# laboshinl/loam_velodyne

Measured on AMD Instinct MI355X. Metric: sweeps/sec (64-ring, 1M-pt map): feature extraction + odometry + scan-to-map registration, higher is better.
Workload: dtype f32

## Files before the change

### loam_velodyne_amd/csrc/gn_iter_kernel.inc

```
__global__ __launch_bounds__(LX_RES_THREADS) __attribute__((amdgpu_waves_per_eu(GN_WAVES, GN_WAVES))) void GN_KERNEL(const GnArgs A) {
  constexpr int TRS = GN_TILE + 1;
  __shared__ uint32_t s_raw[(36 * GN_TILE > LX_NSUM * TRS) ? 36 * GN_TILE : LX_NSUM * TRS];
  float* tr = (float*)s_raw;
  uint32_t* s_tab = s_raw;
  __shared__ uint32_t s_nb[5 * GN_TILE];
  __shared__ double red[8][LX_NSUM];
  __shared__ int sh_last;
  const uint32_t s = blockIdx.y;
  if (A.stats[s].done) return;
  if (A.skip_word && *A.skip_word == A.skip_value) return;
  const int tid = (int)threadIdx.x;
  const uint32_t q0 = A.ds_off[2 * s], qm = A.ds_off[2 * s + 1], q1 = A.ds_off[2 * s + 2];
  const uint32_t tc = (qm - q0 + GN_TILE - 1) / GN_TILE, tsf = (q1 - qm + GN_TILE - 1) / GN_TILE;
  const uint32_t ntiles = (tc + tsf) ? tc + tsf : 1u;
  uint32_t tile;
  {
    const uint32_t x = blockIdx.x % 8, j = blockIdx.x / 8;
    const uint32_t tsurf = ntiles - tc;
    const uint32_t c0 = x * tc / 8, c1 = (x + 1) * tc / 8, s0 = x * tsurf / 8, s1 = (x + 1) * tsurf / 8;
    if (j < c1 - c0) tile = c0 + j;
    else if (j - (c1 - c0) < s1 - s0) tile = tc + s0 + (j - (c1 - c0));
    else return;
  }
  const bool corner = tile < tc;
  const uint32_t qbase = corner ? q0 + tile * GN_TILE : qm + (tile - tc) * GN_TILE;
  const uint32_t qend = corner ? qm : q1;
  GN_TS(0);
  const Pose T = A.poses[s];
  {
    const int grp = tid / KNN_LPQ, gl = tid % KNN_LPQ;
    const uint32_t q = qbase + (uint32_t)grp;
    if (q < qend) {
      const float4 po = A.ds_pts[q];
      float qx = po.x, qy = po.y, qz = po.z;
      to_map(T, qx, qy, qz);
      unsigned long long wk[6];
      uint32_t win[6];
      knn5_group<KNN_LPQ, GN_TILE>(corner ? *A.cdesc : *A.sdesc, corner ? A.cpts : A.spts, corner ? A.cstart : A.sstart, qx, qy, qz, gl, s_tab + grp, wk,
                                   win);
      if (gl == 0) {
        const float d5 = wk[4] != KNN_NONE ? __uint_as_float((uint32_t)(wk[4] >> 32)) : FLT_MAX;
#pragma unroll
        for (int j = 0; j < 5; j++) s_nb[j * GN_TILE + grp] = (j == 4 && !(d5 < 1.0f)) ? 0xffffffffu : win[j];
      }
    }
  }
// ... 70 lines not shown
```

### loam_velodyne_amd/csrc/odometry.hip

```cpp
#include "odometry.hpp"
#include "odom_schedule.hpp"
#include "pinned_copy.hpp"
#include <chrono>
#include <cstring>
#include <type_traits>

namespace loamx {

constexpr int OD_THREADS = 256;
constexpr int OD_TR_STRIDE = OD_THREADS + 2;
constexpr int OD_PART_STRIDE = 2 * (2 * 16 * LX_NSUM) + 16;
[[maybe_unused]] constexpr int OD_PART_TS = 2 * (2 * 16 * LX_NSUM);

__device__ inline void sincos_f(float a, float& s, float& c) { sincosf(a, &s, &c); }

__device__ inline void transform_to_start(const float* T, float scan_period, const float4 pi, float& x, float& y, float& z) {
  const float s = (1.f / scan_period) * (pi.w - (float)(int)pi.w);
  x = pi.x - s * T[3];
  y = pi.y - s * T[4];
  z = pi.z - s * T[5];
  float sx, cx, sy, cy, sz, cz;
  sincos_f(-s * T[0], sx, cx);
  sincos_f(-s * T[1], sy, cy);
  sincos_f(-s * T[2], sz, cz);
// ... 162 lines not shown
    const uint32_t w = __float_as_uint(p.w);
    if (valid && (d2 < lbest || (d2 == lbest && lw != 0xffffffffu && (w & OD_IDX_MASK) < (lw & OD_IDX_MASK)))) { lbest = d2; lw = w; }
  });
  float d = lbest;
  int j = lw == 0xffffffffu ? -1 : (int)(lw & OD_IDX_MASK), o_ = lw == 0xffffffffu ? 0x7fffffff : (int)(lw & OD_IDX_MASK);
  int ring = (int)(lw >> 24);
  {
#pragma unroll
    for (int off = 32; off > 0; off >>= 1) {
      const float od = __shfl_xor(d, off, 64);
      const int oj = __shfl_xor(j, off, 64), oo = __shfl_xor(o_, off, 64), orr = __shfl_xor(ring, off, 64);
      if (od < d || (od == d && oo < o_)) { d = od; j = oj; o_ = oo; ring = orr; }
    }
  }
  const float h = 1.0f / g.inv_h;
  if (j >= 0 && d < 25.0f && d <= h * h) { w_out = ((uint32_t)ring << 24) | (uint32_t)j; return j; }
  const int id = nn1_shells(g, sorted, cell_start, qx, qy, qz, lane, 2, (j >= 0 && d < 25.0f) ? d : 25.0f, (j >= 0 && d < 25.0f) ? j : -1);
  w_out = id == j ? (((uint32_t)ring << 24) | (uint32_t)j) : (0xff000000u | (uint32_t)(id < 0 ? 0 : id));
  return id;
}

#ifdef LOAMX_PROF_CORR
__device__ unsigned long long g_corr_ts[3][16];
#define OC_TS(k) do { if (blockIdx.y == 0 && lane == 0 && ts_slot >= 0) g_corr_ts[ts_slot][k] = wall_clock64(); } while (0)
#else
#define OC_TS(k) do { } while (0)
#endif
__global__ __launch_bounds__(256) OD_CORR_ATTR void k_odom_corr_grid(OdomProblem* __restrict__ probs, OdomParams P, uint32_t* __restrict__ patch_dst, uint4 patch) {
  if (patch_dst && blockIdx.x == 0 && blockIdx.y == 0 && threadIdx.x == 0) { patch_dst[0] = patch.x; patch_dst[1] = patch.y; patch_dst[2] = patch.z; }
  OdomProblem& pb = probs[blockIdx.y];
  if (pb.done) return;
  const int lane = threadIdx.x & 63, wid = threadIdx.x >> 6;
  const int nSharp = (int)pb.n_sharp, nFlat = (int)pb.n_flat;
  int f;
  {
    const int x = (int)(blockIdx.x % 8), j = (int)(blockIdx.x / 8);
    const int sS = (int)((long long)x * nSharp / 8), nS = (int)((long long)(x + 1) * nSharp / 8) - sS;
    const int sF = (int)((long long)x * nFlat / 8), nF = (int)((long long)(x + 1) * nFlat / 8) - sF;
    const int fl = 4 * j + wid;
    if (fl >= nS + nF) return;
    f = fl < nS ? sS + fl : nSharp + sF + (fl - nS);
  }
#ifdef LOAMX_PROF_CORR
  const int ts_slot = f == nSharp / 2 ? 0 : f == nSharp + nFlat / 2 ? 1 : f == nSharp + nFlat - 1 ? 2 : -1;
#endif
  OC_TS(0);
  float T[6];
#pragma unroll
  for (int k = 0; k < 6; k++) T[k] = pb.transform[k];
  const bool corner = f < nSharp;
  const float4 pi = corner ? pb.sharp[f] : pb.flat[f - nSharp];
  const uint32_t* __restrict__ tbl = corner ? pb.rf_corner : pb.rf_surf;
  const int e0 = max((int)pi.w - 8, 0);
  uint32_t tv = 0u, unordered_epoch = 0u;
  if (tbl) {
    if (e0 + lane < OD_RF_N - 1) tv = tbl[e0 + lane];
    unordered_epoch = tbl[OD_RF_N - 1];
  }
  float x, y, z;
  transform_to_start(T, P.scan_period, pi, x, y, z);
  const GridDescB gd = corner ? *pb.lc_desc : *pb.ls_desc;
  const float4* __restrict__ sorted = pb.sorted;
  const uint32_t* __restrict__ cell_start = pb.cell_table + gd.cell_base;
  OC_TS(1);
  Block27 B;
  block27_build(gd.g, cell_start, x, y, z, lane, B);
  OC_TS(2);
  uint32_t wbest = 0u;
  Block27First first;
  const int closest = nn1_block(gd.g, B, sorted, cell_start, x, y, z, lane, wbest, first);
  OC_TS(3);
  if (closest < 0) {
    if (lane == 0) { pb.ind[5 * f] = -1; pb.ind[5 * f + 1] = -1; pb.ind[5 * f + 2] = -1; }
    return;
  }
  const float4* last = corner ? pb.last_corner : pb.last_surf;
  const int nLast = corner ? (int)pb.n_last_corner : (int)pb.n_last_surf;
  const int nCur = corner ? nSharp : nFlat;
  const int bound = nCur < nLast ? nCur : nLast;
  const int cscan = (wbest >> 24) != 255u ? (int)(wbest >> 24) : (int)last[closest].w;
  float d2 = 25.f, d3 = 25.f;
  int j2 = -1, j3 = -1, o2 = 0x7fffffff, o3 = 0x7fffffff;
  auto better = [](float d, int order, float dbest, int obest) { return d < dbest || (d == dbest && obest != 0x7fffffff && order < obest); };

  bool via_block = false;
  if (tbl && unordered_epoch != pb.rf_epoch && cscan < 255 && B.total > 0u) {
    const unsigned long long valid = __ballot(e0 + lane < OD_RF_N - 1 && (tv >> 24) == pb.rf_epoch);
    auto first_from = [&](int ring) -> int {
      const int k = ring - e0;
      if (k >= 64) return nLast;
      const unsigned long long m = k <= 0 ? valid : (valid >> k) << k;
      if (!m) return nLast;
      const int w = (int)((uint32_t)__shfl((int)tv, __builtin_ctzll(m), 64) & OD_IDX_MASK);
      return w < nLast ? w : nLast;
    };
    if (cscan - 2 >= e0 || e0 == 0) {
// ... 96 lines not shown
            if (corner) {
              if (ring < cscan && better(d, order, d2, o2)) { d2 = d; j2 = j; o2 = order; }
            } else {
              if (ring >= cscan) { if (better(d, order, d2, o2)) { d2 = d; j2 = j; o2 = order; } }
              else { if (better(d, order, d3, o3)) { d3 = d; j3 = j; o3 = order; } }
            }
          }
          if (mb) stop = true;
        }
        baseB -= 256;
        stopB = stop || baseB < 0;
      }
    }
    wave_argmin(d2, j2, o2);
    if (!corner) wave_argmin(d3, j3, o3);
  }
  OC_TS(6);
  if (lane == 0) {
    pb.ind[5 * f] = closest;
    pb.ind[5 * f + 1] = j2;
    pb.ind[5 * f + 2] = corner ? -1 : j3;
  }
#ifdef LOAMX_PROF_CORR
  if (blockIdx.y == 0 && lane == 0 && ts_slot >= 0) {
    g_corr_ts[ts_slot][7] = wall_clock64();
    g_corr_ts[ts_slot][8] = (unsigned long long)B.total; g_corr_ts[ts_slot][9] = (unsigned long long)via_block;
    g_corr_ts[ts_slot][10] = (unsigned long long)closest; g_corr_ts[ts_slot][11] = (unsigned long long)cscan;
  }
#endif
}

#ifdef LOAMX_PROF_LM
#define LM_TS(k) do { if (blockIdx.x == 0 && blockIdx.y == 0 && tid == 0 && iter == it_begin + 1) pb.part[OD_PART_TS + (k)] = (double)wall_clock64(); } while (0)
#else
#define LM_TS(k) do { } while (0)
#endif
#ifndef OD_LM_WAVES
#define OD_LM_WAVES 3
#endif
#ifndef OD_LM_WAVES_MIN
#define OD_LM_WAVES_MIN 3
#endif
#define OD_LM_ATTR __attribute__((amdgpu_waves_per_eu(OD_LM_WAVES_MIN, OD_LM_WAVES)))
#pragma clang diagnostic push
#pragma clang diagnostic ignored "-Wpass-failed"
template <int OD_FPT>
__global__ __launch_bounds__(OD_THREADS) OD_LM_ATTR void k_odom_lm(OdomProblem* __restrict__ probs, OdomParams P, int iter0, int n_iters) {
  OdomProblem& pb = probs[blockIdx.y];
  if (pb.done) return;
  const unsigned NB = gridDim.x;
  const int tid = threadIdx.x;
  const int nSharp = (int)pb.n_sharp, nFlat = (int)pb.n_flat, nFeat = nSharp + nFlat;
// ... 685 lines not shown
      pb.err_word = h_err_.p;
      pb.rf_corner = rf_.p + (size_t)s * OD_RF_N;
      pb.rf_surf = rf_.p + (size_t)(ns + s) * OD_RF_N;
      pb.rf_epoch = rf_epoch_;
      p.max_feat = std::max(p.max_feat, I.n_sharp + I.n_flat);
      p.max_sharp = std::max(p.max_sharp, I.n_sharp);
      p.max_flat = std::max(p.max_flat, I.n_flat);
      p.active.push_back(s);
    }
  }
  if (p.max_feat > 32 * OD_THREADS) throw Error(LOAMX_E_CAPACITY, "more than 8192 sharp+flat features in one sweep");
}

void OdometryBatch::upload_(Pass& p) {
  for (uint32_t s = 0; s < p.ns; s++) h_te_.p[s] = to_end_params(s, p.rc[s] == LOAMX_OK);
  memcpy(h_off_pin_.p, h_cur_off_.data(), sizeof(uint32_t) * (p.K + 1));
  LX_HIP(hipMemcpyAsync(up_dev_.p, up_host_.p, up_bytes_, hipMemcpyHostToDevice, st_));
  index_.prepare(p.K);
  if (!ev_up_) LX_HIP(hipEventCreateWithFlags(&ev_up_, hipEventDisableTiming));
  LX_HIP(hipEventRecord(ev_up_, st_));
  up_pending_ = true;
}

static dim3 odom_corr_grid(uint32_t max_sharp, uint32_t max_flat, uint32_t na) {
  return dim3(8 * (((max_sharp + 7) / 8 + (max_flat + 7) / 8 + 3) / 4), na);
}
OdometryBatch::LmGeometry OdometryBatch::lm_geometry_(uint32_t max_feat) {
#ifdef OD_LM_HALF_WGS
  const uint32_t nb = std::min<uint32_t>(16u, std::max<uint32_t>(1u, (max_feat + 2 * OD_THREADS - 1) / (2 * OD_THREADS)));
#else
  const uint32_t nb = std::min<uint32_t>(16u, (max_feat + OD_THREADS - 1) / OD_THREADS);
#endif
  const bool two = max_feat > nb * OD_THREADS;
  if (!lm_slots_[two]) {
    int per_cu = 0;
    if (two) LX_HIP(hipOccupancyMaxActiveBlocksPerMultiprocessor(&per_cu, k_odom_lm<2>, OD_THREADS, 0));
    else LX_HIP(hipOccupancyMaxActiveBlocksPerMultiprocessor(&per_cu, k_odom_lm<1>, OD_THREADS, 0));
    hipDeviceProp_t prop;
    LX_HIP(hipGetDeviceProperties(&prop, device_));
    lm_slots_[two] = (uint32_t)std::max(per_cu, 1) * (uint32_t)std::max(prop.multiProcessorCount, 1);
  }
  return {nb, two, std::max<uint32_t>(1u, (lm_slots_[two] / 2) / nb)};
}

void OdometryBatch::enqueue_corr_(Pass& p, int k) {
  LtCall* lt = p.lt;
  const int lk = lt && k < LT_MAXP ? k : -1;
  if (lk >= 0) {
    for (int e = 0; e < 3; e++) if (!lt->ev[3 * lk + e]) LX_HIP(hipEventCreate(&lt->ev[3 * lk + e]));
    LX_HIP(hipEventRecord(lt->ev[3 * lk], st_));
  }
  uint32_t* pd = nullptr;
  uint4 pv = make_uint4(0u, 0u, 0u, 0u);
  if (p.patch_pending) { p.patch_pending = false; pd = d_cur_off_.p; pv = make_uint4(h_cur_off_[0], h_cur_off_[1], h_cur_off_[2], 0u); }
  hipLaunchKernelGGL(k_odom_corr_grid, odom_corr_grid(p.max_sharp, p.max_flat, (uint32_t)p.active.size()), dim3(256), 0, st_, prob_.p, params, pd, pv);
  if (lk >= 0) LX_HIP(hipEventRecord(lt->ev[3 * lk + 1], st_));
}
void OdometryBatch::enqueue_lm_(Pass& p, int k) {
  LtCall* lt = p.lt;
  const uint32_t na = (uint32_t)p.active.size();
  const int it0 = 5 * k;
  const int nit = std::min(5, params.max_iterations - it0);
  const int lk = lt && k < LT_MAXP ? k : -1;
  const LmGeometry g = lm_geometry_(p.max_feat);
  for (uint32_t a0 = 0; a0 < na; a0 += g.chunk) {
    const uint32_t nc = std::min(g.chunk, na - a0);
    if (g.two) hipLaunchKernelGGL(k_odom_lm<2>, dim3(g.nb, nc), dim3(OD_THREADS), 0, st_, prob_.p + a0, params, it0, nit);
    else hipLaunchKernelGGL(k_odom_lm<1>, dim3(g.nb, nc), dim3(OD_THREADS), 0, st_, prob_.p + a0, params, it0, nit);
  }
  if (lk >= 0) { LX_HIP(hipEventRecord(lt->ev[3 * lk + 2], st_)); lt->pairs = lk + 1; }
}

struct OdometryBatch::PairOps {
  OdometryBatch& o; Pass& p;
  void corr(int k) { o.enqueue_corr_(p, k); }
  void lm(int k) { o.enqueue_lm_(p, k); }
  void after_first() { o.resolve_late_(p); }
  bool behind(int want) const {
// ... 47 lines not shown
    float4* q = cur_.p; size_t c = cur_.cap;
    DevBuf<float4>& oldest = older_[keep_ - 2];
    cur_.p = oldest.p; cur_.cap = oldest.cap;
    for (int k = keep_ - 2; k > 0; k--) { older_[k].p = older_[k - 1].p; older_[k].cap = older_[k - 1].cap; }
    older_[0].p = last_.p; older_[0].cap = last_.cap;
    last_.p = q; last_.cap = c;
  }
  h_last_off_ = h_cur_off_;
  index_.build(last_.p, h_last_off_.data(), p.K, d_cur_off_.p, fuse_bounds && p.n_all > 0);
  if (!ev_tail_) LX_HIP(hipEventCreateWithFlags(&ev_tail_, hipEventDisableTiming));
  LX_HIP(hipEventRecord(ev_tail_, st_));
  tail_pending_ = true;
}

void OdometryBatch::prof_print_() {
#ifdef LOAMX_PROF_CORR
  unsigned long long ts[3][16];
  LX_HIP(hipMemcpyFromSymbol(ts, HIP_SYMBOL(g_corr_ts), sizeof(ts)));
  for (int q = 0; q < 3; q++)
    fprintf(stderr, "[corr ts %s, us since entry] feature+trig %.2f block table %.2f nn1 %.2f decision %.2f block windows %.2f walk %.2f end %.2f | block %llu pts, via block %llu, closest %lld cscan %lld\n",
            q == 0 ? "corner" : q == 1 ? "flat mid" : "flat last", (ts[q][1] - ts[q][0]) * 0.01, (ts[q][2] - ts[q][0]) * 0.01, (ts[q][3] - ts[q][0]) * 0.01,
            (ts[q][4] - ts[q][0]) * 0.01, (ts[q][5] - ts[q][0]) * 0.01, (ts[q][6] - ts[q][0]) * 0.01, (ts[q][7] - ts[q][0]) * 0.01, ts[q][8], ts[q][9],
            (long long)ts[q][10], (long long)ts[q][11]);
#endif
#ifdef LOAMX_PROF_LM
  double tl[16];
  LX_HIP(hipMemcpy(tl, part_.p + OD_PART_TS, sizeof(tl), hipMemcpyDeviceToHost));
  fprintf(stderr, "[lm ts, 10ns ticks]");
  for (int k = 1; k < 10; k++) fprintf(stderr, " %d:%+.0f", k, tl[k] - tl[0]);
  fprintf(stderr, "\n");
#endif
}

void OdometryBatch::collect_(Pass& p) {
  const uint32_t na = (uint32_t)p.active.size();
  wait_event(ev_pose_);
  if (*(volatile uint32_t*)h_err_.p) {
    *h_err_.p = 0u;
    throw Error(LOAMX_E_HIP, "odometry: the exchange between a stream's k_odom_lm workgroups timed out (not all of them resident)");
  }
  prof_print_();
  int need = 1;
  for (uint32_t a = 0; a < na; a++) need = std::max(need, (h_mirror_.p[a].stats.iterations + 4) / 5);
  pred_pairs_ = need;
  for (uint32_t a = 0; a < na; a++) {
    OdomStream& S = *streams_[p.active[a]];
// ... 158 lines not shown
```

### loam_velodyne_amd/csrc/registration.hip

```cpp
#include "registration.hpp"
#include "pinned_copy.hpp"
#include <atomic>
#include <chrono>
#include "scan.hpp"
#include "voxel.hpp"

namespace loamx {

__global__ __launch_bounds__(256) void k_stack(const float4* __restrict__ in, const float4* const* __restrict__ src, uint32_t n,
                                               const uint32_t* __restrict__ seg_off, uint32_t nseg, const Pose* __restrict__ poses,
                                               float inv_corner, float inv_surf, float4* __restrict__ stack, int* __restrict__ ijk,
                                               int* __restrict__ seg_minmax) {
  const uint32_t i = blockIdx.x * blockDim.x + threadIdx.x;
  const bool active = i < n;
  uint32_t seg = 0;
  int ix = 0, iy = 0, iz = 0;
  if (active) {
    seg = vox_find_seg(seg_off, nseg, i);
    const Pose T = poses[seg >> 1];
    const float4 p = src ? src[seg][i - seg_off[seg]] : in[i];
    float x = p.x, y = p.y, z = p.z;
    to_map(T, x, y, z);
    to_be_mapped(T, x, y, z);
    stack[i] = make_float4(x, y, z, p.w);
// ... 401 lines not shown
    for (int k = 0; k < 6; k++) { bk[k] = gl == 0 ? wk[k] : KNN_NONE; bp[k] = win[k]; }
    knn_scan_group<9, KNN_MLP, LPQ>(pts, beg, len, qx, qy, qz, gl, bk, bp);
  }
  knn_pop6<LPQ>(bk, bp, gl, wk, win);
}

struct GnArgs {
  const float4* ds_pts;
  const uint32_t* ds_off;
  Pose* poses;
  SweepStats* stats;
  const GridDesc* cdesc;
  const float4* cpts;
  const uint32_t* cstart;
  const GridDesc* sdesc;
  const float4* spts;
  const uint32_t* sstart;
  double* partials;
  uint32_t* arrive;
  float* matP;
  SweepStats* host_stats;
  Pose* host_poses;
  uint32_t nblk;
  unsigned long long* dbg;
  int iter;
  float delta_t_abort, delta_r_abort;
  const uint32_t* skip_word;
  uint32_t skip_value;
};

constexpr int GN_TILE = LX_RES_THREADS / KNN_LPQ;
#ifdef LOAMX_PROF_GN
#define GN_TS(k) do { if (blockIdx.y == 0 && tid == 0 && A.iter == 0) A.dbg[(size_t)tile * 8 + (k)] = wall_clock64(); } while (0)
#else
#define GN_TS(k) do { } while (0)
#endif

#ifndef GN_WAVES
#define GN_WAVES 6
#endif
#define GN_KERNEL k_gn_iter
#define GN_JACOBI false
#include "gn_iter_kernel.inc"
#undef GN_KERNEL
#undef GN_JACOBI
#ifdef LOAMX_DIAG
#define GN_KERNEL k_gn_iter_jacobi
#define GN_JACOBI true
#include "gn_iter_kernel.inc"
#undef GN_KERNEL
#undef GN_JACOBI
#endif

__global__ __launch_bounds__(256) void k_knn_probe(const float4* __restrict__ queries, uint32_t n, const GridDesc* __restrict__ desc,
                                                   const float4* __restrict__ pts, const uint32_t* __restrict__ cell_start,
                                                   uint32_t* __restrict__ idx5, float* __restrict__ d2_5) {
// ... 155 lines not shown
  LX_REQUIRE(next_staged_, "swap_submap() without a staged sub-map");
  LX_HIP(hipSetDevice(device_));
  LX_HIP(hipStreamWaitEvent(st_, ev_build_, 0));
  LX_HIP(hipEventRecord(ev_swap_, st_));
  corner_index.swap(corner_next_);
  surf_index.swap(surf_next_);
  corner_index.bind(st_);
  surf_index.bind(st_);
  next_staged_ = false;
  swapped_once_ = true;
}

template <class Count> static void prefix_offsets(std::vector<uint32_t>& off, uint32_t n, Count&& count) {
  off.assign(n + 1, 0);
  for (uint32_t s = 0; s < n; s++) off[s + 1] = off[s] + count(s);
}

template <class Count> void Registrar::plan_inputs_(uint32_t n_sweeps, bool staged, Count&& count) {
  LX_REQUIRE(n_sweeps >= 1 && n_sweeps <= max_sweeps_, "n_sweeps out of range for this handle");
  LX_HIP(hipSetDevice(device_));
  n_sweeps_ = n_sweeps;
  h_seg_off_.assign(2 * n_sweeps + 1, 0);
  if (!staged) h_full_off_.assign(n_sweeps + 1, 0);
  max_q_per_sweep_ = 0;
  for (uint32_t s = 0; s < n_sweeps; s++) {
    const uint32_t nc = count(s, 0), nf = count(s, 1);
    h_seg_off_[2 * s + 1] = h_seg_off_[2 * s] + nc;
    h_seg_off_[2 * s + 2] = h_seg_off_[2 * s + 1] + nf;
    max_q_per_sweep_ = std::max(max_q_per_sweep_, nc + nf);
    if (!staged) h_full_off_[s + 1] = h_full_off_[s] + count(s, 2);
  }
  n_in_ = h_seg_off_[2 * n_sweeps];
  if (!staged) n_full_ = h_full_off_[n_sweeps];
  in_.reserve(n_in_ + 1);
  stack_.reserve(n_in_ + 1);
  ds_pts_.reserve(n_in_ + 1);
  vox_.reserve(n_in_ + 1, 2 * n_sweeps);
  LX_REQUIRE(n_in_ < SCAN_MAX_N, "too many feature points in one batch");
  if (n_full_) full_.reserve(n_full_);
  nblk_ = max_q_per_sweep_ / GN_TILE + 2;
  partials_.reserve((size_t)n_sweeps * nblk_ * LX_NSUM);
}

size_t Registrar::write_param_block_(const float* guess6, const float4* const* corner_src, const float4* const* surf_src, const float4* const* full_src) {
  const uint32_t ns = n_sweeps_;
  const size_t nseg = 2 * (size_t)ns;
  const size_t o_off = sizeof(float) * 6 * ns, o_full = o_off + sizeof(uint32_t) * (nseg + 1);
  const size_t end_full = o_full + sizeof(uint32_t) * (ns + 1), o_src = (end_full + 15) & ~(size_t)15;
  const size_t bytes = corner_src ? o_src + sizeof(float4*) * (nseg + ns) : end_full;
  h_blob_.reserve(bytes + 16);
  blob_.reserve(bytes + 16);
  memcpy(h_blob_.p, guess6, sizeof(float) * 6 * ns);
// ... 147 lines not shown
        memcpy(&T, (const void*)&h_poses_.p[k], sizeof(T));
        all = st.pad1 == mirror_check_word(st, T);
      }
      if (all) return true;
    }
    if ((spin & 15) == 15) {
      const hipError_t q = hipEventQuery(ev_look_);
      if (q == hipSuccess) return false;
      if (q != hipErrorNotReady) LX_HIP(q);
    }
    cpu_relax();
  }
}

RegOutcome Registrar::run_iterations(RunTrace& tr) {
  TraceRange trace_range("loamx:registration:gauss-newton");
  GnArgs a;
  a.ds_pts = ds_pts_.p; a.ds_off = ds_off_.p; a.poses = poses_.p; a.stats = stats_.p;
  a.cdesc = corner_index.desc(); a.cpts = corner_index.sorted(); a.cstart = corner_index.cell_start();
  a.sdesc = surf_index.desc(); a.spts = surf_index.sorted(); a.sstart = surf_index.cell_start();
  a.partials = partials_.p; a.arrive = arrive_.p; a.matP = matP_.p;
  a.host_stats = h_stats_.p; a.host_poses = h_poses_.p;
  a.nblk = nblk_; a.delta_t_abort = params.delta_t_abort; a.delta_r_abort = params.delta_r_abort;
  a.dbg = nullptr;
  a.skip_word = run_.vb_unchecked ? vb_.d_fail_word() : nullptr;
  a.skip_value = vb_.epoch();
#ifdef LOAMX_PROF_GN
  g_gn_dbg.reserve((size_t)nblk_ * 8 + 64);
  LX_HIP(hipMemsetAsync(g_gn_dbg.p, 0, sizeof(unsigned long long) * ((size_t)nblk_ * 8 + 64), st_));
  a.dbg = g_gn_dbg.p;
#endif
  struct Ops {
    Registrar& r;
    GnArgs& a;
    RunTrace& tr;
    const dim3 grid;
    void gn(int it) {
      const bool tm = r.timing_ && r.launch_timing_ && r.n_res_launch_ < 64;
      if (tm) LX_HIP(hipEventRecord(r.ev_[2 + 2 * r.n_res_launch_], r.st_));
      a.iter = it;
#ifdef LOAMX_DIAG
      if (r.jacobi_eig_) hipLaunchKernelGGL(k_gn_iter_jacobi, grid, dim3(LX_RES_THREADS), 0, r.st_, a);
      else
#endif
      hipLaunchKernelGGL(k_gn_iter, grid, dim3(LX_RES_THREADS), 0, r.st_, a);
      if (tm) {
        LX_HIP(hipEventRecord(r.ev_[3 + 2 * r.n_res_launch_], r.st_));
        r.n_res_launch_++;
      }
    }
    void full(int mode) { r.enqueue_full(mode); }
    void mark() {
      if (tr.on && tr.first_gn == 0) tr.first_gn = host_us();
      if (!r.ev_look_) LX_HIP(hipEventCreateWithFlags(&r.ev_look_, hipEventDisableTiming));
      LX_HIP(hipEventRecord(r.ev_look_, r.st_));
    }
    void first_wait() {
      if (r.on_first_wait) { r.on_first_wait(); r.on_first_wait = nullptr; }
    }
    RegLook look() {
      if (tr.on && tr.callback == 0) tr.callback = host_us();
      r.wait_for_mirrors();
      RegLook l{r.bucket_stage_gave_up_(), true, 0};
      for (uint32_t k = 0; k < r.n_sweeps_ && !l.gave_up; k++) {
        l.all_done = l.all_done && r.h_stats_.p[k].done;
        l.need = std::max(l.need, r.h_stats_.p[k].iterations);
      }
      return l;
    }
  } ops{*this, a, tr, dim3(8 * ((nblk_ + 7) / 8 + 1), n_sweeps_)};
  static const int ahead = diag_env("LOAMX_GN_AHEAD") ? std::max(0, atoi(diag_env("LOAMX_GN_AHEAD"))) : 1;
  const RegOutcome o = reg_schedule(ops, RegPlan{early_exit, params.max_iterations, pred_iters_, ahead, n_full_ != 0 && !defer_full});
  pred_iters_ = o.pred_iters_next;
  run_.mirrors_written = run_.results_final = o.all_done;
  tr.looks = o.looks;
#ifdef LOAMX_PROF_GN
  dump_gn_profile_();
#endif
  return o;
}

#ifdef LOAMX_PROF_GN
void Registrar::dump_gn_profile_() {
  std::vector<unsigned long long> h((size_t)nblk_ * 8);
  (void)hipStreamSynchronize(st_);
  (void)hipMemcpy(h.data(), g_gn_dbg.p, sizeof(unsigned long long) * h.size(), hipMemcpyDeviceToHost);
  unsigned long long t0 = ~0ull;
  for (uint32_t t = 0; t < nblk_; t++) if (h[8 * t]) t0 = std::min(t0, h[8 * t]);
  fprintf(stderr, "[gn iter 0, sweep 0: tile: start / search / rows / reduce us (+solve)]");
  for (uint32_t t = 0; t < nblk_; t++) {
    const unsigned long long* v = &h[8 * t];
    if (!v[0]) continue;
    if (t % 16 == 0 || v[5]) fprintf(stderr, " %u:%.0f/%.0f/%.0f/%.0f", t, (v[0] - t0) * 0.01, (v[1] - v[0]) * 0.01, (v[2] - v[1]) * 0.01, (v[3] - v[2]) * 0.01);
    if (v[5]) fprintf(stderr, "(+solve %.0f, ends at %.0f)", (v[5] - v[4]) * 0.01, (v[5] - t0) * 0.01);
  }
  fprintf(stderr, "\n");
  unsigned long long ts[16];
  (void)hipMemcpyFromSymbol(ts, HIP_SYMBOL(g_solve_ts), sizeof(ts));
  fprintf(stderr, "[solve_sweep, us since entry] partial sums %.1f  sums+AtA %.1f  qr %.1f  projector %.1f  trig %.1f  update+stores %.1f\n", (ts[1] - ts[0]) * 0.01,
          (ts[2] - ts[0]) * 0.01, (ts[3] - ts[0]) * 0.01, (ts[4] - ts[0]) * 0.01, (ts[5] - ts[0]) * 0.01, (ts[6] - ts[0]) * 0.01);
}
#endif

void Registrar::begin_attempt_(bool legacy) {
  if (timing_) LX_HIP(hipEventRecord(ev_[0], st_));
  n_res_launch_ = 0;
  if (early_exit) memset(h_stats_.p, 0, sizeof(SweepStats) * n_sweeps_);
  run_ = Run{};
  run_.vb_unchecked = !legacy && n_in_ > 0;
}

// ... 280 lines not shown
```

### loam_velodyne_amd/csrc/registration.hpp

```cpp
#pragma once
#include <functional>
#include "common.h"
#include "dev_math.hpp"
#include "reg_schedule.hpp"
#include "submap_index.hpp"
#include "voxel.hpp"
#include "voxbucket.hpp"

namespace loamx {

constexpr int LX_RES_THREADS = 256;
constexpr int LX_NSUM = 28;

struct SweepStats {
  int iterations, sel, corner_q, surf_q, degenerate, done, pad0, pad1;
};

__host__ __device__ inline int mirror_check_word(const SweepStats& st, const Pose& T) {
  const unsigned* w = reinterpret_cast<const unsigned*>(&T);
  unsigned x = 0x5bd1e995u ^ (unsigned)st.iterations ^ ((unsigned)st.sel << 8) ^ ((unsigned)st.degenerate << 30);
  for (int i = 0; i < (int)(sizeof(Pose) / 4); i++) x = (x << 5 | x >> 27) ^ w[i];
  return (int)x;
}

// ... 66 lines not shown
  PinBuf<float> h_guess_;
  DevBuf<float4> in_, stack_, ds_pts_, full_, full_alt_;
  DevBuf<uint32_t> ds_off_;
  DevBuf<float> guess_;
  bool full_staged_ = false, full_next_staged_ = false;
  std::vector<uint32_t> next_full_off_;
  hipEvent_t ev_look_ = nullptr;
  PinBuf<float4> h_full_dl_;
  struct Run {
    bool vb_unchecked = false;
    bool mirrors_written = false;
    bool results_final = false;
    int full_dl_sweep = -1;
    void* full_dl_direct = nullptr;
  } run_;
  VoxelPipeline vox_;
  VoxBucket vb_;
  bool vb_disabled_ = false;
  bool jacobi_eig_ = false;
  void enqueue_front(bool legacy);
  void enqueue_full(int mode);
  void redo_if_bucket_path_failed();
  uint32_t n_in_ = 0, n_full_ = 0, max_q_per_sweep_ = 0;
  struct RunTrace;
  template <class Count> void plan_inputs_(uint32_t n_sweeps, bool staged, Count&& count);
  size_t write_param_block_(const float* guess6, const float4* const* corner_src, const float4* const* surf_src, const float4* const* full_src);
  void begin_attempt_(bool legacy);
  RegOutcome run_iterations(RunTrace& tr);
  bool bucket_stage_gave_up_();
  void dump_gn_profile_();
  bool wait_for_mirrors();
  void fetch_results();
  int pred_iters_ = 4;

  DevBuf<Pose> poses_;
  DevBuf<SweepStats> stats_;
  DevBuf<float> matP_;
  DevBuf<double> partials_;
  const float* d_guess_ = nullptr;
  const uint32_t* d_seg_off_ = nullptr;
  const uint32_t* d_full_off_ = nullptr;
  const float4* const* d_src_ = nullptr;
  DevBuf<char> blob_;
  PinBuf<char> h_blob_;
  SubMapIndex corner_next_, surf_next_;
  DevBuf<float4> next_corner_, next_surf_;
  PinBuf<float4> h_next_corner_, h_next_surf_;
  hipStream_t st_build_ = nullptr;
  hipEvent_t ev_build_ = nullptr, ev_swap_ = nullptr;
  bool next_staged_ = false, swapped_once_ = false;
  DevBuf<uint32_t> arrive_;
  DevBuf<uint32_t> full_done_;
  uint32_t full_tag_ = 0;
// ... 10 lines not shown
```

Baseline: 16130.

## Reorder odometry correspondence workgroups long-first by stream and use one-wave workgroups

Adds a launch-order layer that maps a flat 1D grid onto stream, phase and tile slots, so that the long flat-feature correspondence work is dispatched before the short sharp work, grouped per stream. The odometry correspondence kernel is now templated on waves per workgroup and defaults to one-wave (64-thread) workgroups instead of four-wave ones. The GN registration kernel gets the same slot mapping but keeps the legacy order by default. The aim is to cut tail imbalance, where long-running workgroups start late, at the cost of extra index arithmetic, more and smaller workgroups, and per-launch getenv calls. Profiling span instrumentation is added behind compile flags.

```diff
diff --git a/loam_velodyne_amd/csrc/gn_iter_kernel.inc b/loam_velodyne_amd/csrc/gn_iter_kernel.inc
--- a/loam_velodyne_amd/csrc/gn_iter_kernel.inc
+++ b/loam_velodyne_amd/csrc/gn_iter_kernel.inc
@@ -6,22 +6,17 @@
   __shared__ uint32_t s_nb[5 * GN_TILE];
   __shared__ double red[8][LX_NSUM];
   __shared__ int sh_last;
-  const uint32_t s = blockIdx.y;
+  const LoSlot slot = lo_gn_slot(A.launch, blockIdx.y * gridDim.x + blockIdx.x);
+  if (!slot.valid) return;
+  const uint32_t s = slot.stream;
   if (A.stats[s].done) return;
   if (A.skip_word && *A.skip_word == A.skip_value) return;
   const int tid = (int)threadIdx.x;
   const uint32_t q0 = A.ds_off[2 * s], qm = A.ds_off[2 * s + 1], q1 = A.ds_off[2 * s + 2];
   const uint32_t tc = (qm - q0 + GN_TILE - 1) / GN_TILE, tsf = (q1 - qm + GN_TILE - 1) / GN_TILE;
   const uint32_t ntiles = (tc + tsf) ? tc + tsf : 1u;
-  uint32_t tile;
-  {
-    const uint32_t x = blockIdx.x % 8, j = blockIdx.x / 8;
-    const uint32_t tsurf = ntiles - tc;
-    const uint32_t c0 = x * tc / 8, c1 = (x + 1) * tc / 8, s0 = x * tsurf / 8, s1 = (x + 1) * tsurf / 8;
-    if (j < c1 - c0) tile = c0 + j;
-    else if (j - (c1 - c0) < s1 - s0) tile = tc + s0 + (j - (c1 - c0));
-    else return;
-  }
+  const uint32_t tile = lo_gn_tile(slot, tc, ntiles);
+  if (tile == LO_NONE) return;
   const bool corner = tile < tc;
   const uint32_t qbase = corner ? q0 + tile * GN_TILE : qm + (tile - tc) * GN_TILE;
   const uint32_t qend = corner ? qm : q1;
diff --git a/loam_velodyne_amd/csrc/launch_order.hpp b/loam_velodyne_amd/csrc/launch_order.hpp
--- /dev/null
+++ b/loam_velodyne_amd/csrc/launch_order.hpp
@@ -0,0 +1,130 @@
+#pragma once
+#include <cstdint>
+#include <cstring>
+
+#if defined(__HIPCC__)
+#define LO_HD __host__ __device__
+#else
+#define LO_HD
+#endif
+
+namespace loamx {
+
+enum class LaunchOrder : uint32_t { Legacy = 0, LongFirst = 1, LongFirstByStream = 2 };
+
+constexpr LaunchOrder LO_DEFAULT_CORR = LaunchOrder::LongFirstByStream;
+constexpr LaunchOrder LO_DEFAULT_GN = LaunchOrder::Legacy;
+constexpr uint32_t LO_DEFAULT_CORR_WG_WAVES = 1u;
+inline uint32_t corr_wg_waves_from(const char* e) { return !e ? LO_DEFAULT_CORR_WG_WAVES : !strcmp(e, "4") ? 4u : !strcmp(e, "1") ? 1u : LO_DEFAULT_CORR_WG_WAVES; }
+struct LaunchOrders {
+  LaunchOrder corr, gn;
+};
+inline LaunchOrders launch_orders_from(const char* e) {
+  LaunchOrders o{LO_DEFAULT_CORR, LO_DEFAULT_GN};
+  if (!e) return o;
+  static const struct { const char* name; LaunchOrder order; } names[] = {{"legacy", LaunchOrder::Legacy}, {"long-first", LaunchOrder::LongFirst}, {"by-stream", LaunchOrder::LongFirstByStream}};
+  for (const auto& nm : names) {
+    const size_t len = strlen(nm.name);
+    if (strncmp(e, nm.name, len)) continue;
+    if (!e[len]) o.corr = o.gn = nm.order;
+    else if (!strcmp(e + len, "-corr")) o.corr = nm.order;
+    else if (!strcmp(e + len, "-gn")) o.gn = nm.order;
+  }
+  return o;
+}
+
+struct LoGrid {
+  uint32_t x, y;
+};
+constexpr uint32_t LO_SHORT = 0u, LO_LONG = 1u, LO_BOTH = 2u;
+struct LoSlot {
+  bool valid;
+  uint32_t stream;
+  uint32_t phase;
+  uint32_t x, j;
+};
+constexpr uint32_t LO_NONE = 0xffffffffu;
+
+LO_HD inline uint32_t lo_ceil_div(uint32_t a, uint32_t b) { return (a + b - 1u) / b; }
+
+struct CorrLaunch {
+  uint32_t order;
+  uint32_t n_streams;
+  uint32_t max_sharp, max_flat;
+};
+LO_HD inline uint32_t lo_corr_phase_wgs(uint32_t max_n, uint32_t wpw) { return lo_ceil_div(lo_ceil_div(max_n, 8u), wpw); }
+LO_HD inline uint32_t lo_corr_legacy_wgs(const CorrLaunch& L, uint32_t wpw) { return 8u * ((lo_ceil_div(L.max_sharp, 8u) + lo_ceil_div(L.max_flat, 8u) + wpw - 1u) / wpw); }
+LO_HD inline LoGrid odom_corr_grid(const CorrLaunch& L, uint32_t wpw) {
+  if (L.order == (uint32_t)LaunchOrder::Legacy) return LoGrid{lo_corr_legacy_wgs(L, wpw), L.n_streams};
+  return LoGrid{8u * L.n_streams * (lo_corr_phase_wgs(L.max_flat, wpw) + lo_corr_phase_wgs(L.max_sharp, wpw)), 1u};
+}
+LO_HD inline LoSlot lo_corr_slot(const CorrLaunch& L, uint32_t wpw, uint32_t b) {
+  if (L.order == (uint32_t)LaunchOrder::Legacy) {
+    const uint32_t per = lo_corr_legacy_wgs(L, wpw), bx = b % per;
+    return LoSlot{b / per < L.n_streams, b / per, LO_BOTH, bx % 8u, bx / 8u};
+  }
+  const uint32_t x = b % 8u, n = L.n_streams;
+  uint32_t q = b / 8u;
+  const uint32_t n_long = n * lo_corr_phase_wgs(L.max_flat, wpw), n_short = n * lo_corr_phase_wgs(L.max_sharp, wpw);
+  const bool by_stream = L.order == (uint32_t)LaunchOrder::LongFirstByStream;
+  if (q < n_long) return by_stream ? LoSlot{true, q / (n_long / n), LO_LONG, x, q % (n_long / n)} : LoSlot{true, q % n, LO_LONG, x, q / n};
+  q -= n_long;
+  if (q < n_short) return by_stream ? LoSlot{true, q / (n_short / n), LO_SHORT, x, q % (n_short / n)} : LoSlot{true, q % n, LO_SHORT, x, q / n};
+  return LoSlot{false, 0u, LO_SHORT, x, 0u};
+}
+LO_HD inline int lo_corr_feature(const LoSlot& s, uint32_t wpw, uint32_t wid, int nSharp, int nFlat) {
+  const int x = (int)s.x, j = (int)s.j;
+  const int sS = (int)((long long)x * nSharp / 8), nS = (int)((long long)(x + 1) * nSharp / 8) - sS;
+  const int sF = (int)((long long)x * nFlat / 8), nF = (int)((long long)(x + 1) * nFlat / 8) - sF;
+  const int fl = (int)wpw * j + (int)wid;
+  if (s.phase == LO_BOTH) {
+    if (fl >= nS + nF) return -1;
+    return fl < nS ? sS + fl : nSharp + sF + (fl - nS);
+  }
+  if (s.phase == LO_LONG) return fl < nF ? nSharp + sF + fl : -1;
+  return fl < nS ? sS + fl : -1;
+}
+
+struct GnLaunch {
+  uint32_t order;
+  uint32_t n_sweeps;
+  uint32_t nblk;
+  uint32_t max_corner_tiles, max_surf_tiles;
+};
+LO_HD inline GnLaunch gn_launch(LaunchOrder order, uint32_t n_sweeps, uint32_t nblk, uint32_t max_corner_pts, uint32_t max_surf_pts, uint32_t tile) {
+  const uint32_t ts = lo_ceil_div(max_surf_pts, tile);
+  return GnLaunch{(uint32_t)order, n_sweeps, nblk, lo_ceil_div(max_corner_pts, tile), ts ? ts : 1u};
+}
+LO_HD inline uint32_t lo_gn_legacy_wgs(const GnLaunch& L) { return 8u * ((L.nblk + 7u) / 8u + 1u); }
+LO_HD inline LoGrid gn_iter_grid(const GnLaunch& L) {
+  if (L.order == (uint32_t)LaunchOrder::Legacy) return LoGrid{lo_gn_legacy_wgs(L), L.n_sweeps};
+  return LoGrid{8u * L.n_sweeps * (lo_ceil_div(L.max_corner_tiles, 8u) + lo_ceil_div(L.max_surf_tiles, 8u)), 1u};
+}
+LO_HD inline LoSlot lo_gn_slot(const GnLaunch& L, uint32_t b) {
+  if (L.order == (uint32_t)LaunchOrder::Legacy) {
+    const uint32_t per = lo_gn_legacy_wgs(L), bx = b % per;
+    return LoSlot{b / per < L.n_sweeps, b / per, LO_BOTH, bx % 8u, bx / 8u};
+  }
+  const uint32_t x = b % 8u, n = L.n_sweeps;
+  uint32_t q = b / 8u;
+  const uint32_t n_long = n * lo_ceil_div(L.max_corner_tiles, 8u), n_short = n * lo_ceil_div(L.max_surf_tiles, 8u);
+  const bool by_stream = L.order == (uint32_t)LaunchOrder::LongFirstByStream;
+  if (q < n_long) return by_stream ? LoSlot{true, q / (n_long / n), LO_LONG, x, q % (n_long / n)} : LoSlot{true, q % n, LO_LONG, x, q / n};
+  q -= n_long;
+  if (q < n_short) return by_stream ? LoSlot{true, q / (n_short / n), LO_SHORT, x, q % (n_short / n)} : LoSlot{true, q % n, LO_SHORT, x, q / n};
+  return LoSlot{false, 0u, LO_SHORT, x, 0u};
+}
+LO_HD inline uint32_t lo_gn_tile(const LoSlot& s, uint32_t tc, uint32_t ntiles) {
+  const uint32_t x = s.x, j = s.j;
+  const uint32_t tsurf = ntiles - tc;
+  const uint32_t c0 = x * tc / 8, c1 = (x + 1) * tc / 8, s0 = x * tsurf / 8, s1 = (x + 1) * tsurf / 8;
+  if (s.phase == LO_BOTH) {
+    if (j < c1 - c0) return c0 + j;
+    if (j - (c1 - c0) < s1 - s0) return tc + s0 + (j - (c1 - c0));
+    return LO_NONE;
+  }
+  if (s.phase == LO_LONG) return j < c1 - c0 ? c0 + j : LO_NONE;
+  return j < s1 - s0 ? tc + s0 + j : LO_NONE;
+}
+
+}
diff --git a/loam_velodyne_amd/csrc/odometry.hip b/loam_velodyne_amd/csrc/odometry.hip
--- a/loam_velodyne_amd/csrc/odometry.hip
+++ b/loam_velodyne_amd/csrc/odometry.hip
@@ -1,5 +1,6 @@
 #include "odometry.hpp"
 #include "odom_schedule.hpp"
+#include "launch_order.hpp"
 #include "pinned_copy.hpp"
 #include <chrono>
 #include <cstring>
@@ -208,28 +209,33 @@
 
 #ifdef LOAMX_PROF_CORR
 __device__ unsigned long long g_corr_ts[3][16];
-#define OC_TS(k) do { if (blockIdx.y == 0 && lane == 0 && ts_slot >= 0) g_corr_ts[ts_slot][k] = wall_clock64(); } while (0)
+#define OC_TS(k) do { if (slot.stream == 0 && lane == 0 && ts_slot >= 0) g_corr_ts[ts_slot][k] = wall_clock64(); } while (0)
+constexpr int OC_SPAN_STREAMS = 16;
+constexpr int OC_SPAN_WORDS = 1 + 4 * OC_SPAN_STREAMS;
+__device__ unsigned long long g_corr_span[OC_SPAN_WORDS + 1];
+#define OC_SPAN_BEGIN() do { if (lane == 0 && (unsigned long long)probs == g_corr_span[OC_SPAN_WORDS]) atomicMin(&g_corr_span[0], (unsigned long long)wall_clock64()); } while (0)
+#define OC_SPAN_END() do { if (lane == 0 && (unsigned long long)probs == g_corr_span[OC_SPAN_WORDS] && slot.stream < (uint32_t)OC_SPAN_STREAMS) { const unsigned long long t_ = wall_clock64(); \
+    unsigned long long* e_ = &g_corr_span[1 + 4 * slot.stream + (f < nSharp ? 0 : 2)]; atomicMin(e_, t_); atomicMax(e_ + 1, t_); } } while (0)
 #else
 #define OC_TS(k) do { } while (0)
+#define OC_SPAN_BEGIN() do { } while (0)
+#define OC_SPAN_END() do { } while (0)
 #endif
-__global__ __launch_bounds__(256) OD_CORR_ATTR void k_odom_corr_grid(OdomProblem* __restrict__ probs, OdomParams P, uint32_t* __restrict__ patch_dst, uint4 patch) {
-  if (patch_dst && blockIdx.x == 0 && blockIdx.y == 0 && threadIdx.x == 0) { patch_dst[0] = patch.x; patch_dst[1] = patch.y; patch_dst[2] = patch.z; }
-  OdomProblem& pb = probs[blockIdx.y];
+template <int WG_WAVES> __global__ __launch_bounds__(64 * WG_WAVES) OD_CORR_ATTR void k_odom_corr_grid(OdomProblem* __restrict__ probs, OdomParams P, const CorrLaunch L, uint32_t* __restrict__ patch_dst, uint4 patch) {
+  const uint32_t wg = blockIdx.y * gridDim.x + blockIdx.x;
+  if (patch_dst && wg == 0 && threadIdx.x == 0) { patch_dst[0] = patch.x; patch_dst[1] = patch.y; patch_dst[2] = patch.z; }
+  const LoSlot slot = lo_corr_slot(L, WG_WAVES, wg);
+  if (!slot.valid) return;
+  OdomProblem& pb = probs[slot.stream];
   if (pb.done) return;
   const int lane = threadIdx.x & 63, wid = threadIdx.x >> 6;
   const int nSharp = (int)pb.n_sharp, nFlat = (int)pb.n_flat;
-  int f;
-  {
-    const int x = (int)(blockIdx.x % 8), j = (int)(blockIdx.x / 8);
-    const int sS = (int)((long long)x * nSharp / 8), nS = (int)((long long)(x + 1) * nSharp / 8) - sS;
-    const int sF = (int)((long long)x * nFlat / 8), nF = (int)((long long)(x + 1) * nFlat / 8) - sF;
-    const int fl = 4 * j + wid;
-    if (fl >= nS + nF) return;
-    f = fl < nS ? sS + fl : nSharp + sF + (fl - nS);
-  }
+  const int f = lo_corr_feature(slot, WG_WAVES, (uint32_t)wid, nSharp, nFlat);
+  if (f < 0) return;
 #ifdef LOAMX_PROF_CORR
   const int ts_slot = f == nSharp / 2 ? 0 : f == nSharp + nFlat / 2 ? 1 : f == nSharp + nFlat - 1 ? 2 : -1;
 #endif
+  OC_SPAN_BEGIN();
   OC_TS(0);
   float T[6];
 #pragma unroll
@@ -258,6 +264,7 @@
   OC_TS(3);
   if (closest < 0) {
     if (lane == 0) { pb.ind[5 * f] = -1; pb.ind[5 * f + 1] = -1; pb.ind[5 * f + 2] = -1; }
+    OC_SPAN_END();
     return;
   }
   const float4* last = corner ? pb.last_corner : pb.last_surf;
@@ -400,12 +407,13 @@
     pb.ind[5 * f + 2] = corner ? -1 : j3;
   }
 #ifdef LOAMX_PROF_CORR
-  if (blockIdx.y == 0 && lane == 0 && ts_slot >= 0) {
+  if (slot.stream == 0 && lane == 0 && ts_slot >= 0) {
     g_corr_ts[ts_slot][7] = wall_clock64();
     g_corr_ts[ts_slot][8] = (unsigned long long)B.total; g_corr_ts[ts_slot][9] = (unsigned long long)via_block;
     g_corr_ts[ts_slot][10] = (unsigned long long)closest; g_corr_ts[ts_slot][11] = (unsigned long long)cscan;
   }
 #endif
+  OC_SPAN_END();
 }
 
 #ifdef LOAMX_PROF_LM
@@ -1137,9 +1145,6 @@
   up_pending_ = true;
 }
 
-static dim3 odom_corr_grid(uint32_t max_sharp, uint32_t max_flat, uint32_t na) {
-  return dim3(8 * (((max_sharp + 7) / 8 + (max_flat + 7) / 8 + 3) / 4), na);
-}
 OdometryBatch::LmGeometry OdometryBatch::lm_geometry_(uint32_t max_feat) {
 #ifdef OD_LM_HALF_WGS
   const uint32_t nb = std::min<uint32_t>(16u, std::max<uint32_t>(1u, (max_feat + 2 * OD_THREADS - 1) / (2 * OD_THREADS)));
@@ -1158,6 +1163,12 @@
   return {nb, two, std::max<uint32_t>(1u, (lm_slots_[two] / 2) / nb)};
 }
 
+#ifdef LOAMX_PROF_CORR
+static unsigned long long g_corr_span_host[8][OC_SPAN_WORDS];
+static uint32_t g_corr_span_order[8], g_corr_span_wgs[8];
+static int g_corr_span_launches = 0;
+static std::atomic<const void*> g_corr_span_owner_host{nullptr};
+#endif
 void OdometryBatch::enqueue_corr_(Pass& p, int k) {
   LtCall* lt = p.lt;
   const int lk = lt && k < LT_MAXP ? k : -1;
@@ -1168,7 +1179,32 @@
   uint32_t* pd = nullptr;
   uint4 pv = make_uint4(0u, 0u, 0u, 0u);
   if (p.patch_pending) { p.patch_pending = false; pd = d_cur_off_.p; pv = make_uint4(h_cur_off_[0], h_cur_off_[1], h_cur_off_[2], 0u); }
-  hipLaunchKernelGGL(k_odom_corr_grid, odom_corr_grid(p.max_sharp, p.max_flat, (uint32_t)p.active.size()), dim3(256), 0, st_, prob_.p, params, pd, pv);
+  const CorrLaunch L{(uint32_t)launch_orders_from(getenv("LOAMX_LAUNCH_ORDER")).corr, (uint32_t)p.active.size(), p.max_sharp, p.max_flat};
+  const uint32_t wpw = corr_wg_waves_from(getenv("LOAMX_CORR_WG_WAVES"));
+  const LoGrid g = odom_corr_grid(L, wpw);
+#ifdef LOAMX_PROF_CORR
+  {
+    const void* none = nullptr;
+    const void* mine = prob_.p;
+    const unsigned long long key = (unsigned long long)mine;
+    if (g_corr_span_owner_host.compare_exchange_strong(none, mine))
+      LX_HIP(hipMemcpyToSymbol(HIP_SYMBOL(g_corr_span), &key, sizeof(key), sizeof(unsigned long long) * OC_SPAN_WORDS, hipMemcpyHostToDevice));
+  }
+  const bool span_mine = g_corr_span_owner_host.load() == (const void*)prob_.p;
+  static unsigned long long span_init[OC_SPAN_WORDS];
+  span_init[0] = ~0ull;
+  for (int i = 0; i < 2 * OC_SPAN_STREAMS; i++) { span_init[1 + 2 * i] = ~0ull; span_init[2 + 2 * i] = 0ull; }
+  if (span_mine) LX_HIP(hipMemcpyToSymbolAsync(HIP_SYMBOL(g_corr_span), span_init, sizeof(span_init), 0, hipMemcpyHostToDevice, st_));
+#endif
+  if (wpw == 1) hipLaunchKernelGGL(k_odom_corr_grid<1>, dim3(g.x, g.y), dim3(64), 0, st_, prob_.p, params, L, pd, pv);
+  else hipLaunchKernelGGL(k_odom_corr_grid<4>, dim3(g.x, g.y), dim3(256), 0, st_, prob_.p, params, L, pd, pv);
+#ifdef LOAMX_PROF_CORR
+  if (span_mine && k >= 0 && k < 8) {
+    LX_HIP(hipMemcpyFromSymbolAsync(g_corr_span_host[k], HIP_SYMBOL(g_corr_span), sizeof(g_corr_span_host[k]), 0, hipMemcpyDeviceToHost, st_));
+    g_corr_span_order[k] = L.order | (wpw << 8); g_corr_span_wgs[k] = g.x * g.y;
+    g_corr_span_launches = std::max(g_corr_span_launches, k + 1);
+  }
+#endif
   if (lk >= 0) LX_HIP(hipEventRecord(lt->ev[3 * lk + 1], st_));
 }
 void OdometryBatch::enqueue_lm_(Pass& p, int k) {
@@ -1262,6 +1298,21 @@
             q == 0 ? "corner" : q == 1 ? "flat mid" : "flat last", (ts[q][1] - ts[q][0]) * 0.01, (ts[q][2] - ts[q][0]) * 0.01, (ts[q][3] - ts[q][0]) * 0.01,
             (ts[q][4] - ts[q][0]) * 0.01, (ts[q][5] - ts[q][0]) * 0.01, (ts[q][6] - ts[q][0]) * 0.01, (ts[q][7] - ts[q][0]) * 0.01, ts[q][8], ts[q][9],
             (long long)ts[q][10], (long long)ts[q][11]);
+  LX_HIP(hipStreamSynchronize(st_));
+  for (int k = 0; g_corr_span_owner_host.load() == (const void*)prob_.p && k < g_corr_span_launches; k++) {
+    const unsigned long long* v = g_corr_span_host[k];
+    if (v[0] == ~0ull) continue;
+    static const char* const names[] = {"legacy", "long-first", "by-stream"};
+    fprintf(stderr, "[corr span launch %d order %s waves/wg %u wgs %u]", k, names[g_corr_span_order[k] & 3u], g_corr_span_order[k] >> 8, g_corr_span_wgs[k]);
+    for (int s = 0; s < OC_SPAN_STREAMS; s++) {
+      const unsigned long long* e = v + 1 + 4 * s;
+      if (e[1] == 0ull && e[3] == 0ull) continue;
+      fprintf(stderr, " s%d sharp %.1f..%.1f flat %.1f..%.1f", s, e[1] ? (e[0] - v[0]) * 0.01 : -1.0, e[1] ? (e[1] - v[0]) * 0.01 : -1.0, e[3] ? (e[2] - v[0]) * 0.01 : -1.0,
+              e[3] ? (e[3] - v[0]) * 0.01 : -1.0);
+    }
+    fprintf(stderr, "\n");
+  }
+  if (g_corr_span_owner_host.load() == (const void*)prob_.p) g_corr_span_launches = 0;
 #endif
 #ifdef LOAMX_PROF_LM
   double tl[16];
diff --git a/loam_velodyne_amd/csrc/registration.hip b/loam_velodyne_amd/csrc/registration.hip
--- a/loam_velodyne_amd/csrc/registration.hip
+++ b/loam_velodyne_amd/csrc/registration.hip
@@ -1,5 +1,6 @@
 #include "registration.hpp"
 #include "pinned_copy.hpp"
+#include "launch_order.hpp"
 #include <atomic>
 #include <chrono>
 #include "scan.hpp"
@@ -447,6 +448,7 @@
   SweepStats* host_stats;
   Pose* host_poses;
   uint32_t nblk;
+  GnLaunch launch;
   unsigned long long* dbg;
   int iter;
   float delta_t_abort, delta_r_abort;
@@ -456,7 +458,7 @@
 
 constexpr int GN_TILE = LX_RES_THREADS / KNN_LPQ;
 #ifdef LOAMX_PROF_GN
-#define GN_TS(k) do { if (blockIdx.y == 0 && tid == 0 && A.iter == 0) A.dbg[(size_t)tile * 8 + (k)] = wall_clock64(); } while (0)
+#define GN_TS(k) do { if (tid == 0 && A.iter == 0) A.dbg[((size_t)s * A.nblk + tile) * 8 + (k)] = wall_clock64(); } while (0)
 #else
 #define GN_TS(k) do { } while (0)
 #endif
@@ -658,12 +660,14 @@
   n_sweeps_ = n_sweeps;
   h_seg_off_.assign(2 * n_sweeps + 1, 0);
   if (!staged) h_full_off_.assign(n_sweeps + 1, 0);
-  max_q_per_sweep_ = 0;
+  max_q_per_sweep_ = max_corner_in_ = max_surf_in_ = 0;
   for (uint32_t s = 0; s < n_sweeps; s++) {
     const uint32_t nc = count(s, 0), nf = count(s, 1);
     h_seg_off_[2 * s + 1] = h_seg_off_[2 * s] + nc;
     h_seg_off_[2 * s + 2] = h_seg_off_[2 * s + 1] + nf;
     max_q_per_sweep_ = std::max(max_q_per_sweep_, nc + nf);
+    max_corner_in_ = std::max(max_corner_in_, nc);
+    max_surf_in_ = std::max(max_surf_in_, nf);
     if (!staged) h_full_off_[s + 1] = h_full_off_[s] + count(s, 2);
   }
   n_in_ = h_seg_off_[2 * n_sweeps];
@@ -857,12 +861,14 @@
   a.partials = partials_.p; a.arrive = arrive_.p; a.matP = matP_.p;
   a.host_stats = h_stats_.p; a.host_poses = h_poses_.p;
   a.nblk = nblk_; a.delta_t_abort = params.delta_t_abort; a.delta_r_abort = params.delta_r_abort;
+  a.launch = gn_launch(launch_orders_from(getenv("LOAMX_LAUNCH_ORDER")).gn, n_sweeps_, nblk_, max_corner_in_, max_surf_in_, GN_TILE);
+  const LoGrid lg = gn_iter_grid(a.launch);
   a.dbg = nullptr;
   a.skip_word = run_.vb_unchecked ? vb_.d_fail_word() : nullptr;
   a.skip_value = vb_.epoch();
 #ifdef LOAMX_PROF_GN
-  g_gn_dbg.reserve((size_t)nblk_ * 8 + 64);
-  LX_HIP(hipMemsetAsync(g_gn_dbg.p, 0, sizeof(unsigned long long) * ((size_t)nblk_ * 8 + 64), st_));
+  g_gn_dbg.reserve((size_t)n_sweeps_ * nblk_ * 8 + 64);
+  LX_HIP(hipMemsetAsync(g_gn_dbg.p, 0, sizeof(unsigned long long) * ((size_t)n_sweeps_ * nblk_ * 8 + 64), st_));
   a.dbg = g_gn_dbg.p;
 #endif
   struct Ops {
@@ -903,25 +909,41 @@
       }
       return l;
     }
-  } ops{*this, a, tr, dim3(8 * ((nblk_ + 7) / 8 + 1), n_sweeps_)};
+  } ops{*this, a, tr, dim3(lg.x, lg.y)};
   static const int ahead = diag_env("LOAMX_GN_AHEAD") ? std::max(0, atoi(diag_env("LOAMX_GN_AHEAD"))) : 1;
   const RegOutcome o = reg_schedule(ops, RegPlan{early_exit, params.max_iterations, pred_iters_, ahead, n_full_ != 0 && !defer_full});
   pred_iters_ = o.pred_iters_next;
   run_.mirrors_written = run_.results_final = o.all_done;
   tr.looks = o.looks;
 #ifdef LOAMX_PROF_GN
-  dump_gn_profile_();
+  dump_gn_profile_(a.launch.order);
 #endif
   return o;
 }
 
 #ifdef LOAMX_PROF_GN
-void Registrar::dump_gn_profile_() {
-  std::vector<unsigned long long> h((size_t)nblk_ * 8);
+void Registrar::dump_gn_profile_(uint32_t order) {
+  std::vector<unsigned long long> h((size_t)n_sweeps_ * nblk_ * 8);
+  std::vector<uint32_t> off(2 * (size_t)n_sweeps_ + 1);
   (void)hipStreamSynchronize(st_);
   (void)hipMemcpy(h.data(), g_gn_dbg.p, sizeof(unsigned long long) * h.size(), hipMemcpyDeviceToHost);
+  (void)hipMemcpy(off.data(), ds_off_.p, sizeof(uint32_t) * off.size(), hipMemcpyDeviceToHost);
   unsigned long long t0 = ~0ull;
-  for (uint32_t t = 0; t < nblk_; t++) if (h[8 * t]) t0 = std::min(t0, h[8 * t]);
+  for (size_t t = 0; t < (size_t)n_sweeps_ * nblk_; t++) if (h[8 * t]) t0 = std::min(t0, h[8 * t]);
+  fprintf(stderr, "[gn span iter 0 order %s]", order == 0 ? "legacy" : order == 1 ? "long-first" : "by-stream");
+  for (uint32_t s = 0; s < n_sweeps_; s++) {
+    const uint32_t tc = (off[2 * s + 1] - off[2 * s] + GN_TILE - 1) / GN_TILE;
+    unsigned long long lo[2] = {~0ull, ~0ull}, hi[2] = {0ull, 0ull};
+    for (uint32_t t = 0; t < nblk_; t++) {
+      const unsigned long long e = h[((size_t)s * nblk_ + t) * 8 + 3];
+      if (!e) continue;
+      const int k = t < tc ? 0 : 1;
+      lo[k] = std::min(lo[k], e); hi[k] = std::max(hi[k], e);
+    }
+    fprintf(stderr, " s%u corner %.1f..%.1f surf %.1f..%.1f", s, hi[0] ? (lo[0] - t0) * 0.01 : -1.0, hi[0] ? (hi[0] - t0) * 0.01 : -1.0, hi[1] ? (lo[1] - t0) * 0.01 : -1.0,
+            hi[1] ? (hi[1] - t0) * 0.01 : -1.0);
+  }
+  fprintf(stderr, "\n");
   fprintf(stderr, "[gn iter 0, sweep 0: tile: start / search / rows / reduce us (+solve)]");
   for (uint32_t t = 0; t < nblk_; t++) {
     const unsigned long long* v = &h[8 * t];
diff --git a/loam_velodyne_amd/csrc/registration.hpp b/loam_velodyne_amd/csrc/registration.hpp
--- a/loam_velodyne_amd/csrc/registration.hpp
+++ b/loam_velodyne_amd/csrc/registration.hpp
@@ -112,13 +112,14 @@
   void enqueue_full(int mode);
   void redo_if_bucket_path_failed();
   uint32_t n_in_ = 0, n_full_ = 0, max_q_per_sweep_ = 0;
+  uint32_t max_corner_in_ = 0, max_surf_in_ = 0;
   struct RunTrace;
   template <class Count> void plan_inputs_(uint32_t n_sweeps, bool staged, Count&& count);
   size_t write_param_block_(const float* guess6, const float4* const* corner_src, const float4* const* surf_src, const float4* const* full_src);
   void begin_attempt_(bool legacy);
   RegOutcome run_iterations(RunTrace& tr);
   bool bucket_stage_gave_up_();
-  void dump_gn_profile_();
+  void dump_gn_profile_(uint32_t order);
   bool wait_for_mirrors();
   void fetch_results();
   int pred_iters_ = 4;
```

New measurement: 15580. -3.4%, worse.
